# AbbVie-ComputationalGenomics/SAIGEgds

Hardware: AMD Instinct MI355X
Metric: variants/sec seqAssocGLMM_SPA at N=430K; achieved HBM GB/s vs roofline (higher is better)
Workload: dtype f64

## Files before the change

### saigegds_amd/csrc/host_lanes.h

```cpp
extern "C" int sgx_set_option(sgx_handle *h, const char *name, long long value)
{
	if (!h || !name) return fail(SGX_EINVAL, "sgx_set_option: NULL argument");
	const std::string n(name);
	if (n == "score_v1") h->force_v1 = value != 0;
	else if (n == "force_dense") h->force_dense = value != 0;
	else if (n == "spa_exact") h->force_exact = value != 0;
	else if (n == "pipe_mb") { if (value < 0 || value > 65536) return fail(SGX_EINVAL, "pipe_mb out of range"); h->pipe_bytes = (size_t)value << 20; return SGX_OK; }
	else if (n == "spa_abl") h->spa_abl = (int)value;
	else if (n == "guard_exp") { if (value < 0 || value > 300) return fail(SGX_EINVAL, "guard_exp must be 0..300"); h->guard_tol = std::pow(10.0, -(double)value); }
	else if (n == "three_plane") { if (value < -1 || value > 1) return fail(SGX_EINVAL, "three_plane must be -1 (automatic), 0 or 1"); h->dense_opt = (int)value; return SGX_OK; }
	else if (n == "lanes") {
		if (value < 1 || value > 4) return fail(SGX_EINVAL, "lanes must be 1..4");
		if (h->owner) return fail(SGX_EINVAL, "lanes: not on a twin");
		int rc = sgx_sync(h);
		if (rc) return rc;
		for (int i = (int)value - 1; i < 3; i++) if (h->twins[i]) { sgx_free(h->twins[i]); h->twins[i] = nullptr; }
		for (int i = 0; i < (int)value - 1; i++) {
			if (h->twins[i]) continue;
			sgx_handle *t = new sgx_handle();
			t->device = h->device; t->md = h->md; t->mf_ok = h->mf_ok; t->mfe = h->mfe;
			for (int g = 0; g < MF_MAXG; g++) { t->mf[g] = h->mf[g]; t->mf_nbfv[g] = h->mf_nbfv[g]; }
			t->dF = h->dF; t->dX = h->dX; t->dy = h->dy; t->dmu = h->dmu; t->dmu2 = h->dmu2; t->dXM = h->dXM; t->dFl = h->dFl; t->dQ = h->dQ;
			t->shares_model = true; t->owner = h;
			t->force_dense = h->force_dense; t->force_v1 = h->force_v1; t->force_exact = h->force_exact;
			t->spa_abl = h->spa_abl; t->guard_tol = h->guard_tol;
			rc = set_dev(t);
			if (!rc) rc = alloc_workspace(t);
			if (rc) { sgx_free(t); return rc; }
			h->twins[i] = t;
		}
		h->n_lanes = (int)value; h->next_lane = 0; h->last_issued = nullptr;
		return SGX_OK;
	}
	else return fail(SGX_EINVAL, "sgx_set_option: unknown option '%s'", name);
	for (sgx_handle *t : h->twins) if (t) { int rc = sgx_set_option(t, name, value); if (rc) return rc; }
	return SGX_OK;
}

static int sync_lane(sgx_handle *h)
{
	int rc = set_dev(h);
	if (rc) return rc;
	HIPCHK(hipStreamSynchronize(h->stream));
	if (h->pend_dense.active) {
		h->pend_dense.active = false;
		if (h->stats_pending && h->h_counters[2] > 0) {
			rc = launch_pending_dense(h);
			if (rc) return rc;
			HIPCHK(hipStreamSynchronize(h->stream));
		}
	}
	if (h->stats_pending) {
		h->stats.n_spa = (uint64_t)(h->h_counters[0] + h->h_counters[7] - h->h_counters[6] + h->h_counters[5]);
		h->stats.n_valid = (uint64_t)h->h_counters[1];
		h->stats.n_spa_dense = (uint64_t)h->h_counters[2];
		h->stats.n_spa_slow = (uint64_t)h->h_counters[4];
		h->stats.three_plane = h->used_miss ? 1u : 0u;
		h->stats.n_guarded = (uint32_t)h->h_counters[21];
		h->stats.n_unlisted = (uint32_t)h->h_counters[23] - h->stats.n_guarded;
		if (h->chain_ran) {
			sgx_handle *p = h->owner ? h->owner : h;
			const double frac = 64.0 * (double)h->h_counters[22] / ((double)std::max<uint64_t>(1, h->stats.n_variants) * (double)h->md.N);
			const bool over = (uint64_t)h->stats.n_unlisted * 32 > h->stats.n_variants;
			if (!h->used_miss && (frac > SGX_DENSE_ON || over)) p->dense_mode = true;
			else if (h->used_miss && frac < SGX_DENSE_OFF) p->dense_mode = false;
		}
#ifdef SPA5_PROF
		fprintf(stderr, "routing: tier A %d, tier B %d (of them handed on by A: %d), per-variant kernels %d (series list %d, exact list %d), dense %d\n",
			h->h_counters[0], h->h_counters[7], h->h_counters[6], h->h_counters[5], h->h_counters[3], h->h_counters[4], h->h_counters[2]);
		fprintf(stderr, "spa5 phases (10 ns ticks summed over variants): series kernel %d variants: stage %d count %d index %d gather %d series %d (sweep %d sum %d solve %d) | exact kernel %d variants: stage %d count %d index %d gather %d - sweeps %d\n",
			h->h_counters[3], h->h_counters[8], h->h_counters[9], h->h_counters[10], h->h_counters[11], h->h_counters[12], h->h_counters[13], h->h_counters[14], h->h_counters[15],
			h->h_counters[4], h->h_counters[16], h->h_counters[17], h->h_counters[18], h->h_counters[19], h->h_counters[21]);
#endif
		float a = 0, b = 0, c = 0;
		(void)hipEventElapsedTime(&a, h->ev[0], h->ev[1]);
		(void)hipEventElapsedTime(&b, h->ev[1], h->ev[2]);
		(void)hipEventElapsedTime(&c, h->ev[0], h->ev[2]);
		h->stats.ms_score = a; h->stats.ms_spa = b; h->stats.ms_total = c;
		float k = 0;
		if (h->evk_set) (void)hipEventElapsedTime(&k, h->evk[0], h->evk[1]);
		h->stats.ms_kernel = k; h->evk_set = false;
		float l = 0;
		if (h->lists_timed) { (void)hipEventElapsedTime(&l, h->ev_lists, h->ev[0]); h->stats.ms_total += l; }
		h->stats.ms_lists = l; h->lists_timed = false;
		h->stats_pending = false;
		sgx_handle *p = h->owner ? h->owner : h;
		const sgx_stats &x = h->stats;
		p->total.n_variants += x.n_variants; p->total.n_valid += x.n_valid; p->total.n_spa += x.n_spa;
		p->total.n_spa_dense += x.n_spa_dense; p->total.n_spa_slow += x.n_spa_slow;
		p->total.ms_score += x.ms_score; p->total.ms_spa += x.ms_spa; p->total.ms_total += x.ms_total; p->total.ms_kernel += x.ms_kernel;
		p->total.ms_lists += x.ms_lists;
		p->total.score_launches += x.score_launches; p->total.spa_launches += x.spa_launches;
		p->total.three_plane += x.three_plane; p->total.n_unlisted += x.n_unlisted; p->total.n_guarded += x.n_guarded;
		p->total_calls++;
	}
	return SGX_OK;
}

extern "C" int sgx_sync(sgx_handle *h)
{
	if (!h) return fail(SGX_EINVAL, "sgx_sync: NULL handle");
	int rc = sync_lane(h);
	for (sgx_handle *t : h->twins) if (!rc && t) rc = sync_lane(t);
	return rc;
}

extern "C" int sgx_get_stats(sgx_handle *h, sgx_stats *st)
{
	if (!h || !st) return fail(SGX_EINVAL, "sgx_get_stats: NULL argument");
	int rc = sgx_sync(h);
	if (rc) return rc;
	*st = (h->last_issued && h->last_issued != h) ? h->last_issued->stats : h->stats;
	return SGX_OK;
}

extern "C" int sgx_get_stats_total(sgx_handle *h, sgx_stats *st, uint64_t *n_calls, int reset)
{
	if (!h || !st) return fail(SGX_EINVAL, "sgx_get_stats_total: NULL argument");
	int rc = sgx_sync(h);
	if (rc) return rc;
	*st = h->total;
	if (n_calls) *n_calls = h->total_calls;
	if (reset) { h->total = sgx_stats{}; h->total_calls = 0; }
	return SGX_OK;
}
```

### saigegds_amd/csrc/host_spa.h

```cpp


#define FOR_EACH_K(X) X(1) X(2) X(3) X(4) X(5) X(6) X(7) X(8) X(9) X(10) X(11) X(12) X(13) X(14) X(15) X(16)

static dim3 mf_grid(int n_cu, size_t rows, int ntile, int *tps, int vpb = MF_VPB, int wg_per_cu = 2)
{
	const int vt = (int)((rows + vpb - 1) / vpb);
	int sk = std::max(1, (n_cu * wg_per_cu * 4 + vt / 2) / vt);
	sk = std::min(sk, std::max(1, ntile / 24));
	if (sk >= 6) sk = (sk + 7) & ~7;
	sk = std::min(sk, std::max(1, ntile / 2));
	*tps = (ntile + sk - 1) / sk;
	*tps += *tps & 1;
	sk = (ntile + *tps - 1) / *tps;
	return dim3((unsigned)vt, (unsigned)sk);
}

template <int INPUT>
static int launch_spa(sgx_handle *h, RowsRef rr, size_t M, double *out8, bool lazy_dense = false)
{
	const DevModel &md = h->md;
	constexpr int PB = 512;
	hipStream_t st = h->stream;
	h->stats.spa_launches = 0;
	if (!md.quant) {
		const dim3 sgrid((unsigned)std::min<size_t>(M, (size_t)h->spa_grid));
		switch (md.K) {
#define MOMENTS(KK, NCX, TIER, RD)                                                               \
	do {                                                                                         \
		if (INPUT == IN_2BIT)                                                                    \
			hipLaunchKernelGGL((spa4_moments<KK, NCX>), dim3((unsigned)h->n_cu), \
				dim3(WAVE * spa4_waves(KK)), fl, st, rr, md, h->nseg,  \
				TIER, btop, (RD) * h->vcap4, h->vcap4, h->recs, h->counters, h->seg4, h->spa_abl, h->cur5 + 2); \
		else                                                                                     \
			hipLaunchKernelGGL((spa4_moments_ds<KK, NCX, (INPUT == IN_2BIT ? IN_U8 : INPUT)>),   \
				dim3((unsigned)h->n_cu), dim3(WAVE * spa4_waves(KK)), fl, st, (const void *)rr.base, rr.bpv, md, \
				h->nseg, TIER, btop, (RD) * h->vcap4, h->vcap4, h->recs, h->counters, h->seg4, h->cur5 + 2);  \
		hipLaunchKernelGGL((spa4_solve<KK, NCX>), gsolve, dim3(256), 0, st, md, h->nseg, TIER,   \
			btop, (RD) * h->vcap4, h->vcap4, h->recs, h->counters, h->seg4, h->fallback,         \
			h->fb_x2, out8, h->force_dense ? 1 : 0, h->force_exact ? 1 : 0);                     \
	} while (0)
#define CASE(KK)                                                                             \
	case KK:                                                                                 \
		if (h->force_v1 && INPUT != IN_2BIT) {                                               \
			hipLaunchKernelGGL((spa_kernel<KK, PB, INPUT>), sgrid, dim3(PB), 0, st, rr,    \
				md, h->recs, h->counters, 0, (const int *)nullptr, h->scratch,    \
				h->scratch_stride, out8);                                                    \
		} else {                                                                             \
			              \
			const size_t fl = spa4_lds_bytes(KK);                                            \
			if (!h->mom_attr_set[INPUT]) {                                                   \
				const void *fa = INPUT == IN_2BIT ? (const void *)spa4_moments<KK, SPA4_NCA> \
					: (const void *)spa4_moments_ds<KK, SPA4_NCA, (INPUT == IN_2BIT ? IN_U8 : INPUT)>; \
				const void *fb = INPUT == IN_2BIT ? (const void *)spa4_moments<KK, SPA4_NCB> \
					: (const void *)spa4_moments_ds<KK, SPA4_NCB, (INPUT == IN_2BIT ? IN_U8 : INPUT)>; \
				HIPCHK(hipFuncSetAttribute(fa, hipFuncAttributeMaxDynamicSharedMemorySize, (int)fl)); \
				HIPCHK(hipFuncSetAttribute(fb, hipFuncAttributeMaxDynamicSharedMemorySize, (int)fl)); \
				h->mom_attr_set[INPUT] = true;                                               \
			}                                                                                \
			const int nround = (int)((M + h->vcap4 - 1) / h->vcap4);                         \
			const int btop = (int)(2 * M);                                                   \
			const dim3 gsolve((unsigned)std::min((h->vcap4 + 3) / 4, 4 * h->n_cu));    \
			                                    \
			 \
			const size_t rowb5 = (size_t)((md.N + 63) / 64) * 16;                            \
			const size_t l5 = (INPUT == IN_2BIT && rowb5 <= 120 * 1024) ? rowb5 : 0;         \
			const bool small5 = INPUT == IN_2BIT && rowb5 <= 32 * 1024;                      \
			if (l5 > 48 * 1024 && !h->spa5_attr_set[INPUT]) {                                \
				HIPCHK(hipFuncSetAttribute((const void *)spa5_kernel<KK, INPUT, 0, 512>,     \
					hipFuncAttributeMaxDynamicSharedMemorySize, (int)l5));                   \
				HIPCHK(hipFuncSetAttribute((const void *)spa5_kernel<KK, INPUT, 1, 512>,     \
					hipFuncAttributeMaxDynamicSharedMemorySize, (int)l5));                   \
				h->spa5_attr_set[INPUT] = true;                                              \
			}                                                                                \
			const int fx5 = (h->force_exact ? 1 : 0) | (h->spa_abl & ~1);                    \
			for (int rd = 0; rd < nround; rd++) MOMENTS(KK, SPA4_NCA, 0, rd);                \
			for (int rd = 0; rd < nround; rd++) MOMENTS(KK, SPA4_NCB, 1, rd);                \
			 \
			const int only5 = (INPUT == IN_2BIT && rr.cptr != nullptr && (h->spa_abl & 512)) ? 2 : 0; \
			const size_t ws5 = spa5_wg_bytes(md.N);                                          \
			if (small5) {                                                                    \
				 \
				constexpr int IN5 = INPUT == IN_2BIT ? INPUT : IN_2BIT;                      \
				hipLaunchKernelGGL((spa5_kernel<KK, IN5, 0, 128>), dim3((unsigned)h->nwg5), dim3(128), \
					l5, st, rr, md, h->recs, h->counters, h->fb_spa2, h->fb_x2, h->cur5, \
					h->fallback, h->scr5, out8, h->force_dense ? 1 : 0, fx5, l5, only5, ws5, 3); \
				hipLaunchKernelGGL((spa5_kernel<KK, IN5, 1, 128>), dim3((unsigned)h->nwg5), dim3(128), \
					l5, st, rr, md, h->recs, h->counters, h->fb_x2, h->fb_x2, h->cur5 + 1, \
					h->fallback, h->scr5, out8, h->force_dense ? 1 : 0, fx5, l5, only5, ws5, 4); \
			} else {                                                                         \
				hipLaunchKernelGGL((spa5_kernel<KK, INPUT, 0, 512>), dim3((unsigned)h->n_cu), dim3(512), \
					l5, st, rr, md, h->recs, h->counters, h->fb_spa2, h->fb_x2, h->cur5, \
					h->fallback, h->scr5, out8, h->force_dense ? 1 : 0, fx5, l5, only5, ws5, 3); \
				hipLaunchKernelGGL((spa5_kernel<KK, INPUT, 1, 512>), dim3((unsigned)h->n_cu), dim3(512), \
					l5, st, rr, md, h->recs, h->counters, h->fb_x2, h->fb_x2, h->cur5 + 1, \
					h->fallback, h->scr5, out8, h->force_dense ? 1 : 0, fx5, l5, only5, ws5, 4); \
			}                                                                                \
			if (!lazy_dense)                                                                 \
				hipLaunchKernelGGL((spa_kernel<KK, PB, INPUT>), sgrid, dim3(PB), 0, st, rr,  \
					md, h->recs, h->counters, 2, h->fallback, h->scratch,                    \
					h->scratch_stride, out8);                                                \
		}                                                                                    \
		break;
			FOR_EACH_K(CASE)
#undef CASE
#undef MOMENTS
		}
		HIPCHK(hipGetLastError());
		h->stats.spa_launches = (h->force_v1 && INPUT != IN_2BIT) ? 1u : (uint32_t)(4 * ((M + h->vcap4 - 1) / h->vcap4) + 3);
		if (lazy_dense && !(h->force_v1 && INPUT != IN_2BIT)) { h->pend_dense.active = true; h->pend_dense.rr = rr; h->pend_dense.M = M; h->pend_dense.out8 = out8; }
	}
	return SGX_OK;
}

static int launch_pending_dense(sgx_handle *h)
{
	const DevModel &md = h->md;
	const RowsRef rr = h->pend_dense.rr;
	double *out8 = h->pend_dense.out8;
	const dim3 sgrid((unsigned)std::min<size_t>(h->pend_dense.M, (size_t)h->spa_grid));
	switch (md.K) {
#define DCASE(KK) case KK: hipLaunchKernelGGL((spa_kernel<KK, 512, IN_2BIT>), sgrid, dim3(512), 0, h->stream, rr, md, h->recs, \
		h->counters, 2, h->fallback, h->scratch, h->scratch_stride, out8); break;
		FOR_EACH_K(DCASE)
#undef DCASE
	}
	HIPCHK(hipGetLastError());
	return SGX_OK;
}

template <int INPUT>
static int launch_scan(sgx_handle *h, const void *rows, size_t row_bytes, size_t M,
	double *out8, uint8_t *valid)
{
	const DevModel &md = h->md;
	constexpr int SB = 256;
	hipStream_t st = h->stream;
	const RowsRef rr{reinterpret_cast<const uint8_t *>(rows), row_bytes, 0, nullptr, nullptr, nullptr};
	HIPCHK(hipMemsetAsync(h->counters, 0, 24 * sizeof(int), st));
	if (h->cur5) HIPCHK(hipMemsetAsync(h->cur5, 0, 8 * sizeof(int), st));
	HIPCHK(hipEventRecord(h->ev[0], st));
	{
	const dim3 grid((unsigned)M);
		switch (md.K) {
	#define CASE(KK)                                                                             \
		case KK:                                                                                 \
			if (INPUT == IN_2BIT)                                                                \
				hipLaunchKernelGGL((score2b_kernel<2 * KK + 2, SB>), grid, dim3(SB), 0, st,     \
					rr, (int)M, md, h->recs, h->counters, out8, valid, (const int *)nullptr, 0, 0, (int *)nullptr, (int *)nullptr); \
			else if (KK <= 8 && !h->force_v1) {                                                  \
				         \
				constexpr int PT = (KK <= 8) ? 2 * KK + 2 : 4;                                   \
				const int vb = (int)((M + DS_TILE_VB - 1) / DS_TILE_VB);                         \
				int ns = std::max(1, std::min((4 * h->n_cu + vb - 1) / vb, (md.N + 4095) / 4096)); \
				int per = (((md.N + ns - 1) / ns) + 63) & ~63;                                   \
				ns = (md.N + per - 1) / per;                                                     \
				const size_t need = (size_t)ns * M * (3 * PT + 2) * sizeof(double);              \
				if (need > h->ds_part_cap) {                                                     \
					HIPCHK(hipStreamSynchronize(st));                                            \
					if (h->ds_part) HIPCHK(hipFree(h->ds_part));                                 \
					h->ds_part = nullptr; h->ds_part_cap = 0;                                    \
					HIPCHK(hipMalloc((void **)&h->ds_part, need));                               \
					h->ds_part_cap = need;                                                       \
				}                                                                                \
				const dim3 gt((unsigned)vb, (unsigned)ns);                                       \
				if (INPUT == IN_U8)                                                              \
					hipLaunchKernelGGL((score_ds_tile_kernel<PT, uint8_t>), gt, dim3(256), 0, st, \
						(const uint8_t *)rows, (int)M, md, per, h->ds_part);                     \
				else                                                                             \
					hipLaunchKernelGGL((score_ds_tile_kernel<PT, double>), gt, dim3(256), 0, st, \
						(const double *)rows, (int)M, md, per, h->ds_part);                      \
				hipLaunchKernelGGL((score_ds_tile_epilogue<PT>), dim3((unsigned)((M + 255) / 256)), dim3(256), 0, st, \
					(int)M, md, ns, h->ds_part, h->recs, h->counters, out8, valid);              \
			} else if (INPUT == IN_U8)                                                           \
				hipLaunchKernelGGL((score_ds_kernel<2 * KK + 2, SB, uint8_t>), grid, dim3(SB), 0, st, \
					(const uint8_t *)rows, (int)M, md, h->recs, h->counters, out8, valid);      \
			else                                                                                 \
				hipLaunchKernelGGL((score_ds_kernel<2 * KK + 2, SB, double>), grid, dim3(SB), 0, st, \
					(const double *)rows, (int)M, md, h->recs, h->counters, out8, valid);       \
			break;
			FOR_EACH_K(CASE)
	#undef CASE
		default: return fail(SGX_EINVAL, "unsupported K=%d", md.K);
		}
	}
	HIPCHK(hipGetLastError());
	HIPCHK(hipEventRecord(h->ev[1], st));
	h->stats.score_launches = 1;
	h->used_miss = false; h->chain_ran = false;
	int rc = launch_spa<INPUT>(h, rr, M, out8);
	if (rc) return rc;
	HIPCHK(hipEventRecord(h->ev[2], st));
	HIPCHK(hipMemcpyAsync(h->h_counters, h->counters, 24 * sizeof(int), hipMemcpyDeviceToHost, st));
	h->stats.n_variants = M;
	h->stats_pending = true;
	return SGX_OK;
}
```

### saigegds_amd/csrc/kern_spa4.h

```cpp
#pragma once
#include "kern_spa4_tab.h"


#ifndef SPA4_WAVES_LOWK
#define SPA4_WAVES_LOWK 8
#endif
__host__ __device__ constexpr int spa4_waves(int K) { return K <= 8 ? SPA4_WAVES_LOWK : 8; }
#define SPA4_NCA 12
#define SPA4_NCB SPA4_NC
#define SPA4_NSMAX (SPA4_NC + 5)
#define SPA4_TAIL_TOL 1e-10

__device__ __forceinline__ double spa4_fma_svv(double a_sgpr, double x, double c_vgpr)
{
	double r;
	asm("v_fma_f64 %0, %1, %2, %3" : "=v"(r) : "s"(a_sgpr), "v"(x), "v"(c_vgpr));
	return r;
}

__device__ __forceinline__ void spa4_max_abs(double &g, double a)
{
	asm("v_max_f64 %0, %0, |%1|" : "+v"(g) : "v"(a));
}

// ... 341 lines not shown
#pragma unroll
			for (int a = 0; a < NS - 1; a++) acc[a] = 0;
			auto dosage = [&](int j) -> double {
				const int i = s_lo + j * WAVE + lane;
				if (i >= N) return 0.0;
				if (INPUT == IN_U8) {
					const uint8_t v = row[i];
					return (v == 0xFF) ? imp : (minus ? 2.0 - (double)v : (double)v);
				} else {
					const double v = reinterpret_cast<const double *>(row)[i];
					return !isfinite(v) ? imp : (minus ? 2.0 - v : v);
				}
			};
			double gn = dosage(0);
			for (int j = 0; j < nstep; j++) {
				const double G = gn;
				if (j + 1 < nstep) gn = dosage(j + 1);
				if (G != 0) {
					const double *x = tab + (size_t)(j * WAVE + lane) * KP;
					double bb = 0;
#pragma unroll
					for (int a = 0; a < K; a++) bb = fma(x[a], c[a], bb);
					const double mui = x[K];
					const double adj = (G - bb) * inv;
					const double u = mui * (1 - mui);
					acc[0] = fma(mui, G, acc[0]);
					acc[1] += bb;
					acc[2] += fmax(adj, 0.0); acc[3] += fmin(adj, 0.0);
					acc[4] = fma(adj, mui, acc[4]);
					acc[5] = fma(adj * adj, u, acc[5]);
					spa4_max_abs(gmax, adj);
					spa4_cum_terms<NC>(adj * ts, u, 1 - 2 * mui, &acc[6]);
				}
			}
			const int idx = wave_reduce_scatter(acc, lane);
			gmax = wave_max_nonneg_to_last(gmax);
			const size_t base = ((size_t)(vb + vl) * nseg + seg) * NS;
			if (!(lane & (NS - 1 > 16 ? 1 : 3)) && idx < NS - 1) segpart[base + idx] = acc[0];
			if (lane == WAVE - 1) segpart[base + (NS - 1)] = gmax;
		}
	}
	spa4_queue_done(cursor);
}

template <int NC>
struct Spa4Series {
	double k1, k2;
	double kp[NC - 2];
	double ts, gmax;
};

template <int NC>
__device__ __forceinline__ bool spa4_eval(const Spa4Series<NC> &S, double xmax, double t, double &K1s, double &K2s, double &K0s)
{
	const double its = 1 / S.ts, tau = t * its;
	double p0 = 0, p1 = 0, p2 = 0;
#pragma unroll
	for (int n = NC; n >= 3; n--) {
		const double kn = S.kp[n - 3];
		p0 = fma(p0, tau, kn);
		p1 = fma(p1, tau, (double)n * kn);
		p2 = fma(p2, tau, (double)(n * (n - 1)) * kn);
	}
	const double tau2 = tau * tau;
	K0s = fma(t, S.k1, fma(0.5 * t * t, S.k2, p0 * tau2 * tau));
	K1s = S.k1 + fma(t, S.k2, p1 * tau2 * its);
	K2s = fma(p2 * tau, its * its, S.k2);
	double tp = tau;
#pragma unroll
	for (int k = 1; k < NC - 3; k++) tp *= tau;
	const double tail = (fabs((double)(NC * (NC - 1)) * S.kp[NC - 3] * tp * tau) +
		fabs((double)((NC - 1) * (NC - 2)) * S.kp[NC - 4] * tp)) * its * its;
	return S.gmax * fabs(t) <= xmax && tail <= SPA4_TAIL_TOL * fabs(K2s) && isfinite(K2s);
}

template <int NC>
__device__ __forceinline__ bool spa4_root(const Spa4Series<NC> &S, double xmax, double q, double NAmu, double NAsigma, RootState &s)
{
	root_begin(s, q, 0, 0);
	root_feed(s, S.k1, S.k2, NAmu, NAsigma, 0.0, true);
	while (s.active) {
		double K1s, K2s, K0s;
		if (!spa4_eval(S, xmax, s.tnew, K1s, K2s, K0s)) return false;
		root_feed(s, K1s, K2s, NAmu, NAsigma, K0s, true);
	}
	return true;
}

template <int K, int NC>
__device__ __forceinline__ void spa4_solve_one(const DevModel &md, int nseg, int tier, int btop, int v0, int vcap, int v, int lane,
	SpaRec *__restrict__ recs, int *__restrict__ counters, const double *__restrict__ segpart,
	int *__restrict__ fb_dense, int *__restrict__ fb_exact, double *__restrict__ out8, int force_dense, int force_exact);

template <int K, int NC>
__global__ void __launch_bounds__(256)
spa4_solve(DevModel md, int nseg, int tier, int btop, int v0, int vcap, SpaRec *__restrict__ recs, int *__restrict__ counters,
	const double *__restrict__ segpart, int *__restrict__ fb_dense, int *__restrict__ fb_exact,
	double *__restrict__ out8, int force_dense, int force_exact)
{
	const int lane = threadIdx.x & (WAVE - 1);
	const int nflag = min(counters[tier ? 7 : 0] - v0, vcap);
	for (int v = (blockIdx.x * blockDim.x + threadIdx.x) / WAVE; v < nflag; v += gridDim.x * blockDim.x / WAVE)
		spa4_solve_one<K, NC>(md, nseg, tier, btop, v0, vcap, v, lane, recs, counters, segpart, fb_dense, fb_exact, out8,
			force_dense, force_exact);
}

template <int K, int NC>
__device__ __forceinline__ void spa4_solve_one(const DevModel &md, int nseg, int tier, int btop, int v0, int vcap, int v, int lane,
	SpaRec *__restrict__ recs, int *__restrict__ counters, const double *__restrict__ segpart,
	int *__restrict__ fb_dense, int *__restrict__ fb_exact, double *__restrict__ out8, int force_dense, int force_exact)
{
	constexpr int NS = NC + 5;
	const int ri = spa4_rec(tier, btop, v0 + v);
	const SpaRec r = recs[ri];
	double a[NS];
#pragma unroll
	for (int x = 0; x < NS; x++) a[x] = 0;
	for (int s = lane; s < nseg; s += WAVE) {
		const double *p = segpart + ((size_t)v * nseg + s) * NS;
#pragma unroll
		for (int x = 0; x < NS - 1; x++) a[x] += p[x];
		a[NS - 1] = fmax(a[NS - 1], p[NS - 1]);
	}
#pragma unroll
	for (int x = 0; x < NS - 1; x++) a[x] = wave_sum(a[x]);
#pragma unroll
	for (int o = 32; o > 0; o >>= 1) a[NS - 1] = fmax(a[NS - 1], __shfl_xor(a[NS - 1], o, WAVE));
	if (lane > 1) return;
	const double inv = 1 / sqrt(r.AC2);
	double xmu_c = 0, xsum_c = 0;
#pragma unroll
	for (int x = 0; x < K; x++) { xmu_c = fma(md.Xmu[x], r.c[x], xmu_c); xsum_c = fma(md.Xsum[x], r.c[x], xsum_c); }
	const double Tstat = r.S * inv;
	const double var2 = r.var2 / r.AC2, var1 = var2 * md.r;
	const double m1 = (a[0] - xmu_c) * inv;
	const double qtilde = Tstat / sqrt(var1) * sqrt(var2) + m1;
	const double sdev = qtilde - m1, qinv = -sdev + m1;
	const double pn_in = d_pchisq1_upper(sdev * sdev / var2);
	if (fabs(qtilde - m1) / sqrt(var2) < 2.0) {
		if (lane == 0) spa_write_row(r, Tstat, var1, pn_in, true, out8);
		return;
	}
	const double nb = (xsum_c - a[1]) * inv;
	const double L = a[2] + fmax(-nb, 0.0), U = a[3] + fmin(-nb, 0.0);
	const double mar = 1e-9 * (fabs(L) + fabs(U) + fabs(qtilde) + fabs(qinv));
	if (force_dense || !(qtilde < L - mar && qtilde > U + mar && qinv < L - mar && qinv > U + mar)) {
		if (lane == 0) fb_dense[atomicAdd(&counters[2], 1)] = ri;
		return;
	}
	Spa4Series<NC> S;
	S.k1 = a[4]; S.k2 = a[5]; S.ts = r.tscale; S.gmax = a[NS - 1];
#pragma unroll
	for (int x = 0; x < NC - 2; x++) S.kp[x] = a[6 + x];
	const double NAmu = m1 - a[4], NAsigma = var2 - a[5];
	const double qmine = lane == 0 ? qtilde : qinv;
	RootState sm;
	const bool ok_mine = !force_exact && spa4_root(S, md.spa_xmax, qmine, NAmu, NAsigma, sm);
	double p_mine = 0;
	if (ok_mine && sm.converged) p_mine = lugannani_rice(sm.root, sm.Kcur, sm.K2cur, qmine, NAmu, NAsigma);
	const int st_mine = (ok_mine ? 1 : 0) | (ok_mine && sm.converged ? 2 : 0);
	const double p_other = __shfl(p_mine, 1, WAVE);
	const int st_other = __shfl(st_mine, 1, WAVE);
	if (lane != 0) return;
	if (!(st_mine & 1) || !(st_other & 1)) {
		if (tier == 0 && !force_exact) {
			const int slot = atomicAdd(&counters[7], 1);
			atomicAdd(&counters[6], 1);
			recs[btop - 1 - slot] = r;
		} else {
			fb_exact[atomicAdd(&counters[4], 1)] = ri;
		}
		return;
	}
	double pval;
	bool converged = true;
	if ((st_mine & 2) && (st_other & 2)) {
		pval = fabs(p_mine) + fabs(p_other);
		if (pval != 0 && pn_in / pval > 1000) pval = pn_in;
	} else {
		pval = pn_in;
		converged = false;
	}
	spa_write_row(r, Tstat, var1, pval, converged, out8);
}


#define SPA5_BIG 2048

__device__ __forceinline__ void cgf_terms_rt(double g, double m, double t, bool with_k, double &k1, double &k2, double &k0)
{
	const double om = 1 - m, mg = m * g, c2 = om * mg * g;
	const double e = fast_exp(-g * t);
	const double d = fma(om, e, m);
	const double rr = isfinite(d) ? fast_rcp(d) : 0.0;
	k1 = fma(mg, rr, k1);
	const double tt = c2 * e * rr * rr;
	if (isfinite(tt)) k2 += tt;
	if (with_k) k0 += cgf_korg_term(g, m, t, d, om);
}

__host__ __device__ inline size_t spa5_wg_bytes(int N) { return (((size_t)N + 63) & ~(size_t)63) * (16 + 4); }

template <int BLOCK>
__device__ __noinline__ void spa5_cum_sweep(const double2 *__restrict__ glist, int nnz, double ts, double *kp_out)
{
	constexpr int NC = SPA4_NCB;
	double kp[NC - 1];
#pragma unroll
	for (int a = 0; a < NC - 1; a++) kp[a] = 0;
	double2 gn = (int)threadIdx.x < nnz ? glist[threadIdx.x] : make_double2(0.0, 0.5);
	for (int k = threadIdx.x; k < nnz; k += BLOCK) {
		const double2 gm = gn;
		if (k + BLOCK < nnz) gn = glist[k + BLOCK];
		const double mui = gm.y;
		spa4_cum_terms<NC>(gm.x * ts, mui * (1 - mui), 1 - 2 * mui, kp);
		kp[NC - 2] = fmax(kp[NC - 2], fabs(gm.x));
	}
#pragma unroll
	for (int a = 0; a < NC - 1; a++) kp_out[a] = kp[a];
}

__device__ __noinline__ int spa5_series_solve(const double *arg, const SpaRec *__restrict__ rec, double *__restrict__ out8)
{
	constexpr int NC = SPA4_NCB;
	Spa4Series<NC> S;
#pragma unroll
	for (int a = 0; a < NC - 2; a++) S.kp[a] = arg[a];
	S.k1 = arg[NC - 2]; S.k2 = arg[NC - 1]; S.ts = arg[NC]; S.gmax = arg[NC + 1];
	const double xmax = arg[NC + 2], qtilde = arg[NC + 3], qinv = arg[NC + 4], NAmu = arg[NC + 5], NAsigma = arg[NC + 6];
	const double pn_in = arg[NC + 7], Tstat = arg[NC + 8], var1 = arg[NC + 9];
	RootState s1, s2;
	if (!spa4_root(S, xmax, qtilde, NAmu, NAsigma, s1) || !spa4_root(S, xmax, qinv, NAmu, NAsigma, s2)) return 0;
	double pval;
	bool converged = true;
	if (s1.converged && s2.converged) {
		const double p1 = lugannani_rice(s1.root, s1.Kcur, s1.K2cur, qtilde, NAmu, NAsigma);
		const double p2 = lugannani_rice(s2.root, s2.Kcur, s2.K2cur, qinv, NAmu, NAsigma);
		pval = fabs(p1) + fabs(p2);
		if (pval != 0 && pn_in / pval > 1000) pval = pn_in;
	} else {
		pval = pn_in;
		converged = false;
	}
	const SpaRec rr = *rec;
	spa_write_row(rr, Tstat, var1, pval, converged, out8);
	return 1;
}

template <int BLOCK>
__device__ __forceinline__ bool spa5_series(const double2 *__restrict__ glist, int nnz, double ts, double xmax,
	double k1, double k2, double qtilde, double qinv, double NAmu, double NAsigma, double pn_in,
	double Tstat, double var1, const SpaRec *__restrict__ rec, double *__restrict__ out8, double *sh, int *sh_flag, int *prof = nullptr)
{
	constexpr int NC = SPA4_NCB;
	double kp[NC - 1];
#ifdef SPA5_PROF
	long long tp_ = wall_clock64();
#define SPA5_TS(ph) do { if (threadIdx.x == 0) { const long long now_ = wall_clock64(); atomicAdd(&prof[ph], (int)(now_ - tp_)); tp_ = now_; } } while (0)
#else
#define SPA5_TS(ph) do { } while (0)
#endif
	spa5_cum_sweep<BLOCK>(glist, nnz, ts, kp);
	SPA5_TS(0);
	constexpr int NWV = BLOCK / WAVE;
	double gmax = kp[NC - 2];
	const int lane = threadIdx.x & (WAVE - 1), wv = threadIdx.x / WAVE;
	double kr[NC - 2];
#pragma unroll
	for (int a = 0; a < NC - 2; a++) kr[a] = kp[a];
	const int idx = wave_reduce_scatter(kr, lane);
#pragma unroll
	for (int o = 32; o > 0; o >>= 1) gmax = fmax(gmax, __shfl_xor(gmax, o, WAVE));
	double *part = sh + NC + 16;
	if (!(lane & 3) && idx < NC - 2) part[idx * NWV + wv] = kr[0];
	if (lane == 1) part[(NC - 2) * NWV + wv] = gmax;
	__syncthreads();
	double *arg = sh;
	if (threadIdx.x < NC - 2) {
		double t = 0;
		for (int w = 0; w < NWV; w++) t += part[threadIdx.x * NWV + w];
		arg[threadIdx.x] = t;
	}
	__syncthreads();
	SPA5_TS(1);
	if (threadIdx.x == 0) {
		for (int w = 0; w < NWV; w++) gmax = fmax(gmax, part[(NC - 2) * NWV + w]);
		arg[NC - 2] = k1; arg[NC - 1] = k2; arg[NC] = ts; arg[NC + 1] = gmax; arg[NC + 2] = xmax;
		arg[NC + 3] = qtilde; arg[NC + 4] = qinv; arg[NC + 5] = NAmu; arg[NC + 6] = NAsigma;
		arg[NC + 7] = pn_in; arg[NC + 8] = Tstat; arg[NC + 9] = var1;
		*sh_flag = spa5_series_solve(arg, rec, out8);
	}
	SPA5_TS(2);
	__syncthreads();
	const bool done = *sh_flag != 0;
	__syncthreads();
	return done;
}

#ifndef SPA5_REG_WAVES
#define SPA5_REG_WAVES 2
#endif
#define SPA5_WAVES_PER_SIMD(BLOCK) ((BLOCK) == 512 ? SPA5_REG_WAVES : ((BLOCK) / 64 + 3) / 4)
#ifdef SPA5_PROF
#define SPA5_T(ph) do { if (tid == 0) { const long long now_ = wall_clock64(); atomicAdd(&counters[8 + 8 * MODE + (ph)], (int)(now_ - tprev_)); tprev_ = now_; } } while (0)
#else
#define SPA5_T(ph) do { } while (0)
#endif
template <int K, int INPUT, int MODE, int BLOCK>
__global__ void __launch_bounds__(BLOCK, SPA5_WAVES_PER_SIMD(BLOCK))
spa5_kernel(RowsRef rr, DevModel md, const SpaRec *__restrict__ recs,
	int *__restrict__ counters, const int *__restrict__ todo, int *__restrict__ todo_next, int *__restrict__ cursor,
	int *__restrict__ fb_dense, uint8_t *__restrict__ scratch, double *__restrict__ out8, int force_dense, int force_exact,
	size_t lds_row_bytes, int only, size_t wg_stride, int nslot)
{
	constexpr int KP = (K + 2) & ~1, NW = BLOCK / WAVE;
	extern __shared__ __attribute__((aligned(16))) uint8_t fill_smem[];
	uint4 *rows_lds = reinterpret_cast<uint4 *>(fill_smem);
	__shared__ double sh[SPA4_NCB * NW + SPA4_NCB + 16];
	__shared__ int sh_flag;
	__shared__ int shi[NW];
	__shared__ int sh_vi, sh_v;
	__shared__ SpaRec sh_rec;
	const int N = md.N, tid = threadIdx.x, lane = tid & (WAVE - 1), wid = tid / WAVE;
	double2 *glist = reinterpret_cast<double2 *>(scratch + (size_t)blockIdx.x * wg_stride);
	uint32_t *ilist = reinterpret_cast<uint32_t *>(glist + (((size_t)N + 63) & ~(size_t)63));
	const int ntodo = counters[nslot];
	const int nvec = INPUT == IN_2BIT ? (int)(min((size_t)((N + 63) >> 6) * 16, rr_row_bytes(rr)) / 16) : (N + 63) >> 6;
	const int per = ((nvec + NW - 1) / NW + WAVE - 1) & ~(WAVE - 1);
	for (;;) {
		__syncthreads();
		if (tid < WAVE) {
			int vi0 = 0;
			if (tid == 0) vi0 = atomicAdd(cursor, 1);
			vi0 = __builtin_amdgcn_readfirstlane(vi0);
			int v0 = -1;
			if (vi0 < 2 * ntodo) {
				v0 = todo[vi0 < ntodo ? vi0 : vi0 - ntodo];
				const double *src = reinterpret_cast<const double *>(recs + v0);
				for (int i = tid; i < (int)(sizeof(SpaRec) / 8); i += WAVE) reinterpret_cast<double *>(&sh_rec)[i] = src[i];
			}
			if (tid == 0) { sh_vi = vi0; sh_v = v0; }
		}
		__syncthreads();
		const int vi = sh_vi;
		if (vi >= 2 * ntodo) break;
#ifdef SPA5_PROF
		long long tprev_ = wall_clock64();
#endif
		const bool big_round = vi < ntodo;
		const int v = sh_v;
		const SpaRec &r = sh_rec;
		if ((r.nnz > SPA5_BIG) != big_round) continue;
		auto row_piece = [&](int p) -> uint4 { return *reinterpret_cast<const uint4 *>(rr.base + rr_piece(rr, (size_t)r.j, (size_t)p)); };
		const uint32_t zx = r.minus ? 0xAAAAAAAAu : 0u;
		const double lut0 = r.lut[0], lut1 = r.lut[1], lut2 = r.lut[2], lut3 = r.lut[3];
		const bool listed = INPUT == IN_2BIT && only != 2 && rr.cptr != nullptr && rr.corient[r.j] == (r.minus ? 2 : 1);
		const uint32_t *il = listed ? rr.cidx + rr.cptr[r.j] : ilist;
		int nnz = listed ? r.nnz : 0;
		if (!listed) {
			const bool staged = INPUT == IN_2BIT && lds_row_bytes >= (size_t)nvec * 16;
			if (staged) {
				constexpr int UN = 8;
				for (int p0 = tid; p0 < nvec; p0 += UN * BLOCK) {
					uint4 t[UN];
	#pragma unroll
					for (int j = 0; j < UN; j++) { const int p = p0 + j * BLOCK; t[j] = p < nvec ? row_piece(p) : make_uint4(0u, 0u, 0u, 0u); }
	#pragma unroll
					for (int j = 0; j < UN; j++) { const int p = p0 + j * BLOCK; if (p < nvec) rows_lds[p] = t[j]; }
				}
				__syncthreads();
			}
			SPA5_T(0);
			auto masks = [&](int p, uint32_t (&ww)[4], uint32_t (&z)[4]) -> int {
				int cnt = 0;
				if (INPUT == IN_2BIT) {
					uint4 w = make_uint4(0u, 0u, 0u, 0u);
					if (p < nvec) w = staged ? rows_lds[p] : row_piece(p);
					ww[0] = w.x; ww[1] = w.y; ww[2] = w.z; ww[3] = w.w;
	#pragma unroll
					for (int k = 0; k < 4; k++) { z[k] = nz_fields((ww[k] ^ zx) & keep_mask(N - p * 64 - 16 * k)); cnt += __popc(z[k]); }
				} else {
					z[0] = z[1] = z[2] = z[3] = 0;
					if (p < nvec) {
						for (int s2 = 0; s2 < 64; s2++) {
							const int i = p * 64 + s2;
							if (i < N && load_dosage<INPUT>(rr, i, r) != 0) { z[s2 >> 5] |= 1u << (s2 & 31); cnt++; }
						}
					}
				}
				return cnt;
			};
			int cnt_w = 0;
			for (int it = 0; it < per; it += WAVE) {
				uint32_t ww[4], z[4];
				cnt_w += masks(wid * per + it + lane, ww, z);
			}
			cnt_w = wave_sum_i(cnt_w);
			if (lane == 0) shi[wid] = cnt_w;
			__syncthreads();
			int o_w = 0;
	#pragma unroll
			for (int w = 0; w < NW; w++) { if (w < wid) o_w += shi[w]; nnz += shi[w]; }
			SPA5_T(1);
			for (int it = 0; it < per; it += WAVE) {
				uint32_t ww[4], z[4];
				const int p = wid * per + it + lane;
				const int cnt = masks(p, ww, z);
				if (!__ballot(cnt != 0)) continue;
				int incl = cnt;
	#pragma unroll
				for (int o = 1; o < WAVE; o <<= 1) {
					const int up = __shfl_up(incl, o, WAVE);
					if (lane >= o) incl += up;
				}
				int o2 = o_w + incl - cnt;
				o_w += __shfl(incl, WAVE - 1, WAVE);
				if (INPUT == IN_2BIT) {
	#pragma unroll
					for (int k = 0; k < 4; k++) {
						uint32_t zz = z[k];
						while (zz) {
							const int b = __ffs(zz) - 1;
							zz &= zz - 1;
							ilist[o2++] = (uint32_t)(p * 64 + 16 * k + (b >> 1)) | (((ww[k] >> b) & 3u) << 30);
						}
					}
				} else {
	#pragma unroll
					for (int k = 0; k < 2; k++) {
						uint32_t zz = z[k];
						while (zz) {
							const int b = __ffs(zz) - 1;
							zz &= zz - 1;
							ilist[o2++] = (uint32_t)(p * 64 + 32 * k + b);
						}
					}
				}
			}
			__syncthreads();
			SPA5_T(2);
		}
		const double inv = 1 / sqrt(r.AC2);
		double c[K];
#pragma unroll
		for (int a = 0; a < K; a++) c[a] = r.c[a];
		double a6[6] = {0, 0, 0, 0, 0, 0};
		constexpr int UNG = K <= 4 ? 4 : 2;
		for (int k0 = tid; k0 < ((force_exact & 128) ? 0 : nnz); k0 += UNG * BLOCK) {
			uint32_t e[UNG];
			double xv[UNG][KP];
#pragma unroll
			for (int j = 0; j < UNG; j++) e[j] = (k0 + j * BLOCK < nnz) ? il[k0 + j * BLOCK] : 0u;
#pragma unroll
			for (int j = 0; j < UNG; j++) {
				const double *x = md.XM + (size_t)(e[j] & 0x3FFFFFFFu) * KP;
#pragma unroll
				for (int a = 0; a < KP; a += 2) {
					const double2 t2 = *reinterpret_cast<const double2 *>(x + a);
					xv[j][a] = t2.x; xv[j][a + 1] = t2.y;
				}
			}
#pragma unroll
			for (int j = 0; j < UNG; j++) {
				const int k = k0 + j * BLOCK;
				if (k >= nnz) continue;
				const uint32_t code = e[j] >> 30;
				const double G = INPUT == IN_2BIT ? ((code & 2u) ? ((code & 1u) ? lut3 : lut2) : ((code & 1u) ? lut1 : lut0))
					: load_dosage<INPUT>(rr, (int)(e[j] & 0x3FFFFFFFu), r);
				double b = 0;
#pragma unroll
				for (int a = 0; a < K; a++) b = fma(xv[j][a], c[a], b);
				const double mui = xv[j][K];
				const double adj = (G - b) * inv;
				glist[k] = make_double2(adj, mui);
				a6[0] = fma(mui, G, a6[0]);
				a6[1] += b;
				if (adj > 0) a6[2] += adj; else a6[3] += adj;
				a6[4] = fma(adj, mui, a6[4]);
				a6[5] = fma(adj * adj, mui * (1 - mui), a6[5]);
			}
		}
		block_sum<6, BLOCK>(a6, sh);
		SPA5_T(3);
		double xmu_c = 0, xsum_c = 0;
#pragma unroll
		for (int a = 0; a < K; a++) { xmu_c = fma(md.Xmu[a], c[a], xmu_c); xsum_c = fma(md.Xsum[a], c[a], xsum_c); }
		const double m1 = (a6[0] - xmu_c) * inv;
		const double Tstat = r.S * inv;
		const double var2 = r.var2 / r.AC2, var1 = var2 * md.r;
		const double qtilde = Tstat / sqrt(var1) * sqrt(var2) + m1;
		const double sdev = qtilde - m1, qinv = -sdev + m1;
		const double pn_in = d_pchisq1_upper(sdev * sdev / var2);
		double pval;
		bool converged = true;
		if (fabs(qtilde - m1) / sqrt(var2) < 2.0) {
			pval = pn_in;
		} else {
			const double nb = (xsum_c - a6[1]) * inv;
			const double L = a6[2] + fmax(-nb, 0.0), U = a6[3] + fmin(-nb, 0.0);
			const double mar = 1e-9 * (fabs(L) + fabs(U) + fabs(qtilde) + fabs(qinv));
			if (force_dense || !(qtilde < L - mar && qtilde > U + mar && qinv < L - mar && qinv > U + mar)) {
				if (tid == 0) fb_dense[atomicAdd(&counters[2], 1)] = v;
				continue;
			}
			const double NAmu = m1 - a6[4], NAsigma = var2 - a6[5];
			if (MODE == 0) {
				if ((force_exact & 1) || !spa5_series<BLOCK>(glist, nnz, r.tscale, md.spa_xmax, a6[4], a6[5], qtilde, qinv, NAmu, NAsigma,
						pn_in, Tstat, var1, &sh_rec, out8, sh, &sh_flag, counters + 13)) {
					if (tid == 0) todo_next[atomicAdd(&counters[4], 1)] = v;
				}
				SPA5_T(4);
				continue;
			}
			RootState s1, s2;
			root_begin(s1, qtilde, L, U);
			root_begin(s2, qinv, L, U);
			root_feed(s1, a6[4], a6[5], NAmu, NAsigma, 0.0, true);
			root_feed(s2, a6[4], a6[5], NAmu, NAsigma, 0.0, true);
			auto sweep = [&](bool a1, bool a2, bool k1w, bool k2w, double t1, double t2, double (&sv)[6]) {
#pragma unroll
				for (int a = 0; a < 6; a++) sv[a] = 0;
				double2 gn = tid < nnz ? glist[tid] : make_double2(0.0, 0.5);
				for (int k0 = tid; k0 < nnz; k0 += BLOCK) {
					const double2 gm = gn;
					if (k0 + BLOCK < nnz) gn = glist[k0 + BLOCK];
					if (a1) cgf_terms_rt(gm.x, gm.y, t1, k1w, sv[0], sv[1], sv[2]);
					if (a2) cgf_terms_rt(gm.x, gm.y, t2, k2w, sv[3], sv[4], sv[5]);
				}
				block_sum<6, BLOCK>(sv, sh);
			};
			while ((s1.active || s2.active) && !(force_exact & 64)) {
				const bool a1 = s1.active, a2 = s2.active, k1w = s1.want_k, k2w = s2.want_k;
				double sv[6];
				sweep(a1, a2, k1w, k2w, s1.tnew, s2.tnew, sv);
				if (a1) root_feed(s1, sv[0], sv[1], NAmu, NAsigma, sv[2], k1w);
				if (a2) root_feed(s2, sv[3], sv[4], NAmu, NAsigma, sv[5], k2w);
			}
			if (s1.converged && s2.converged) {
				if (!(s1.k_ok && s2.k_ok)) {
					double sv[6];
					sweep(!s1.k_ok, !s2.k_ok, true, true, s1.root, s2.root, sv);
					if (!s1.k_ok) s1.Kcur = sv[2];
					if (!s2.k_ok) s2.Kcur = sv[5];
				}
				const double p1 = lugannani_rice(s1.root, s1.Kcur, s1.K2cur, qtilde, NAmu, NAsigma);
				const double p2 = lugannani_rice(s2.root, s2.Kcur, s2.K2cur, qinv, NAmu, NAsigma);
				pval = fabs(p1) + fabs(p2);
				if (pval != 0 && pn_in / pval > 1000) pval = pn_in;
			} else {
				pval = pn_in;
				converged = false;
			}
		}
		if (tid == 0) spa_write_row(r, Tstat, var1, pval, converged, out8);
		SPA5_T(5);
	}
}
```

Measured before the change: 17.64 million.

## Merge series and exact SPA passes into one kernel launch with in-place fallthrough

The two launches of spa5_kernel (series mode, then exact mode over a todo list) become one kernel that reads both the exact and series lists. When the series expansion fails, the variant goes straight to the exact root-finding sweeps in the same workgroup, reusing the already gathered glist and moments instead of re-staging the variant in a second launch. This removes one launch and the repeated gather/count work for the variants that fall through. In exchange, the series and exact paths now share one workgroup's work distribution and can load-imbalance, and a last-block atomic updates counters[4] so the host statistics stay consistent.

Result: no change. 17.70 million, median of 6 (+0.3%).

```diff
diff --git a/saigegds_amd/csrc/host_lanes.h b/saigegds_amd/csrc/host_lanes.h
--- a/saigegds_amd/csrc/host_lanes.h
+++ b/saigegds_amd/csrc/host_lanes.h
@@ -68,9 +68,9 @@
 #ifdef SPA5_PROF
 		fprintf(stderr, "routing: tier A %d, tier B %d (of them handed on by A: %d), per-variant kernels %d (series list %d, exact list %d), dense %d\n",
 			h->h_counters[0], h->h_counters[7], h->h_counters[6], h->h_counters[5], h->h_counters[3], h->h_counters[4], h->h_counters[2]);
-		fprintf(stderr, "spa5 phases (10 ns ticks summed over variants): series kernel %d variants: stage %d count %d index %d gather %d series %d (sweep %d sum %d solve %d) | exact kernel %d variants: stage %d count %d index %d gather %d - sweeps %d\n",
-			h->h_counters[3], h->h_counters[8], h->h_counters[9], h->h_counters[10], h->h_counters[11], h->h_counters[12], h->h_counters[13], h->h_counters[14], h->h_counters[15],
-			h->h_counters[4], h->h_counters[16], h->h_counters[17], h->h_counters[18], h->h_counters[19], h->h_counters[21]);
+		fprintf(stderr, "spa5 phases (10 ns ticks summed over variants): %d variants (series list %d, of them on to the exact sweeps %d): stage %d count %d index %d gather %d series %d (sweep %d sum %d solve %d) exact sweeps %d (%d variants)\n",
+			h->h_counters[3] + h->h_counters[4] - h->h_counters[20], h->h_counters[3], h->h_counters[20], h->h_counters[8], h->h_counters[9], h->h_counters[10],
+			h->h_counters[11], h->h_counters[12], h->h_counters[13], h->h_counters[14], h->h_counters[15], h->h_counters[16], h->h_counters[4]);
 #endif
 		float a = 0, b = 0, c = 0;
 		(void)hipEventElapsedTime(&a, h->ev[0], h->ev[1]);
diff --git a/saigegds_amd/csrc/host_spa.h b/saigegds_amd/csrc/host_spa.h
--- a/saigegds_amd/csrc/host_spa.h
+++ b/saigegds_amd/csrc/host_spa.h
@@ -66,9 +66,7 @@
 			const size_t l5 = (INPUT == IN_2BIT && rowb5 <= 120 * 1024) ? rowb5 : 0;         \
 			const bool small5 = INPUT == IN_2BIT && rowb5 <= 32 * 1024;                      \
 			if (l5 > 48 * 1024 && !h->spa5_attr_set[INPUT]) {                                \
-				HIPCHK(hipFuncSetAttribute((const void *)spa5_kernel<KK, INPUT, 0, 512>,     \
-					hipFuncAttributeMaxDynamicSharedMemorySize, (int)l5));                   \
-				HIPCHK(hipFuncSetAttribute((const void *)spa5_kernel<KK, INPUT, 1, 512>,     \
+				HIPCHK(hipFuncSetAttribute((const void *)spa5_kernel<KK, INPUT, 512>,        \
 					hipFuncAttributeMaxDynamicSharedMemorySize, (int)l5));                   \
 				h->spa5_attr_set[INPUT] = true;                                              \
 			}                                                                                \
@@ -78,22 +76,17 @@
 			 \
 			const int only5 = (INPUT == IN_2BIT && rr.cptr != nullptr && (h->spa_abl & 512)) ? 2 : 0; \
 			const size_t ws5 = spa5_wg_bytes(md.N);                                          \
+			 \
 			if (small5) {                                                                    \
 				 \
 				constexpr int IN5 = INPUT == IN_2BIT ? INPUT : IN_2BIT;                      \
-				hipLaunchKernelGGL((spa5_kernel<KK, IN5, 0, 128>), dim3((unsigned)h->nwg5), dim3(128), \
-					l5, st, rr, md, h->recs, h->counters, h->fb_spa2, h->fb_x2, h->cur5, \
-					h->fallback, h->scr5, out8, h->force_dense ? 1 : 0, fx5, l5, only5, ws5, 3); \
-				hipLaunchKernelGGL((spa5_kernel<KK, IN5, 1, 128>), dim3((unsigned)h->nwg5), dim3(128), \
-					l5, st, rr, md, h->recs, h->counters, h->fb_x2, h->fb_x2, h->cur5 + 1, \
-					h->fallback, h->scr5, out8, h->force_dense ? 1 : 0, fx5, l5, only5, ws5, 4); \
+				hipLaunchKernelGGL((spa5_kernel<KK, IN5, 128>), dim3((unsigned)h->nwg5), dim3(128), \
+					l5, st, rr, md, h->recs, h->counters, h->fb_spa2, h->fb_x2, h->cur5, h->cur5 + 1, \
+					h->fallback, h->scr5, out8, h->force_dense ? 1 : 0, fx5, l5, only5, ws5); \
 			} else {                                                                         \
-				hipLaunchKernelGGL((spa5_kernel<KK, INPUT, 0, 512>), dim3((unsigned)h->n_cu), dim3(512), \
-					l5, st, rr, md, h->recs, h->counters, h->fb_spa2, h->fb_x2, h->cur5, \
-					h->fallback, h->scr5, out8, h->force_dense ? 1 : 0, fx5, l5, only5, ws5, 3); \
-				hipLaunchKernelGGL((spa5_kernel<KK, INPUT, 1, 512>), dim3((unsigned)h->n_cu), dim3(512), \
-					l5, st, rr, md, h->recs, h->counters, h->fb_x2, h->fb_x2, h->cur5 + 1, \
-					h->fallback, h->scr5, out8, h->force_dense ? 1 : 0, fx5, l5, only5, ws5, 4); \
+				hipLaunchKernelGGL((spa5_kernel<KK, INPUT, 512>), dim3((unsigned)h->n_cu), dim3(512), \
+					l5, st, rr, md, h->recs, h->counters, h->fb_spa2, h->fb_x2, h->cur5, h->cur5 + 1, \
+					h->fallback, h->scr5, out8, h->force_dense ? 1 : 0, fx5, l5, only5, ws5); \
 			}                                                                                \
 			if (!lazy_dense)                                                                 \
 				hipLaunchKernelGGL((spa_kernel<KK, PB, INPUT>), sgrid, dim3(PB), 0, st, rr,  \
@@ -106,7 +99,7 @@
 #undef MOMENTS
 		}
 		HIPCHK(hipGetLastError());
-		h->stats.spa_launches = (h->force_v1 && INPUT != IN_2BIT) ? 1u : (uint32_t)(4 * ((M + h->vcap4 - 1) / h->vcap4) + 3);
+		h->stats.spa_launches = (h->force_v1 && INPUT != IN_2BIT) ? 1u : (uint32_t)(4 * ((M + h->vcap4 - 1) / h->vcap4) + 2);
 		if (lazy_dense && !(h->force_v1 && INPUT != IN_2BIT)) { h->pend_dense.active = true; h->pend_dense.rr = rr; h->pend_dense.M = M; h->pend_dense.out8 = out8; }
 	}
 	return SGX_OK;
diff --git a/saigegds_amd/csrc/kern_spa4.h b/saigegds_amd/csrc/kern_spa4.h
--- a/saigegds_amd/csrc/kern_spa4.h
+++ b/saigegds_amd/csrc/kern_spa4.h
@@ -667,16 +667,37 @@
 #endif
 #define SPA5_WAVES_PER_SIMD(BLOCK) ((BLOCK) == 512 ? SPA5_REG_WAVES : ((BLOCK) / 64 + 3) / 4)
 #ifdef SPA5_PROF
-#define SPA5_T(ph) do { if (tid == 0) { const long long now_ = wall_clock64(); atomicAdd(&counters[8 + 8 * MODE + (ph)], (int)(now_ - tprev_)); tprev_ = now_; } } while (0)
+#define SPA5_T(ph) do { if (tid == 0) { const long long now_ = wall_clock64(); atomicAdd(&counters[(ph) == 5 ? 16 : 8 + (ph)], (int)(now_ - tprev_)); tprev_ = now_; } } while (0)
 #else
 #define SPA5_T(ph) do { } while (0)
 #endif
-template <int K, int INPUT, int MODE, int BLOCK>
+struct Spa5Scalars { double m1, Tstat, var2, var1, qtilde, qinv, pn_in, L, U; };
+template <int K>
+__device__ __forceinline__ Spa5Scalars spa5_scalars(const DevModel &md, const SpaRec &r, const double (&a6)[6])
+{
+	Spa5Scalars z;
+	const double inv = 1 / sqrt(r.AC2);
+	double xmu_c = 0, xsum_c = 0;
+#pragma unroll
+	for (int a = 0; a < K; a++) { xmu_c = fma(md.Xmu[a], r.c[a], xmu_c); xsum_c = fma(md.Xsum[a], r.c[a], xsum_c); }
+	z.m1 = (a6[0] - xmu_c) * inv;
+	z.Tstat = r.S * inv;
+	z.var2 = r.var2 / r.AC2; z.var1 = z.var2 * md.r;
+	z.qtilde = z.Tstat / sqrt(z.var1) * sqrt(z.var2) + z.m1;
+	const double sdev = z.qtilde - z.m1;
+	z.qinv = -sdev + z.m1;
+	z.pn_in = d_pchisq1_upper(sdev * sdev / z.var2);
+	const double nb = (xsum_c - a6[1]) * inv;
+	z.L = a6[2] + fmax(-nb, 0.0); z.U = a6[3] + fmin(-nb, 0.0);
+	return z;
+}
+
+template <int K, int INPUT, int BLOCK>
 __global__ void __launch_bounds__(BLOCK, SPA5_WAVES_PER_SIMD(BLOCK))
 spa5_kernel(RowsRef rr, DevModel md, const SpaRec *__restrict__ recs,
-	int *__restrict__ counters, const int *__restrict__ todo, int *__restrict__ todo_next, int *__restrict__ cursor,
-	int *__restrict__ fb_dense, uint8_t *__restrict__ scratch, double *__restrict__ out8, int force_dense, int force_exact,
-	size_t lds_row_bytes, int only, size_t wg_stride, int nslot)
+	int *__restrict__ counters, const int *__restrict__ series, const int *__restrict__ exact, int *__restrict__ cursor,
+	int *__restrict__ done, int *__restrict__ fb_dense, uint8_t *__restrict__ scratch, double *__restrict__ out8, int force_dense,
+	int force_exact, size_t lds_row_bytes, int only, size_t wg_stride)
 {
 	constexpr int KP = (K + 2) & ~1, NW = BLOCK / WAVE;
 	extern __shared__ __attribute__((aligned(16))) uint8_t fill_smem[];
@@ -686,10 +707,11 @@
 	__shared__ int shi[NW];
 	__shared__ int sh_vi, sh_v;
 	__shared__ SpaRec sh_rec;
+	__shared__ double sh_a6[6];
 	const int N = md.N, tid = threadIdx.x, lane = tid & (WAVE - 1), wid = tid / WAVE;
 	double2 *glist = reinterpret_cast<double2 *>(scratch + (size_t)blockIdx.x * wg_stride);
 	uint32_t *ilist = reinterpret_cast<uint32_t *>(glist + (((size_t)N + 63) & ~(size_t)63));
-	const int ntodo = counters[nslot];
+	const int nexact = counters[4], ntodo = nexact + counters[3];
 	const int nvec = INPUT == IN_2BIT ? (int)(min((size_t)((N + 63) >> 6) * 16, rr_row_bytes(rr)) / 16) : (N + 63) >> 6;
 	const int per = ((nvec + NW - 1) / NW + WAVE - 1) & ~(WAVE - 1);
 	for (;;) {
@@ -700,7 +722,8 @@
 			vi0 = __builtin_amdgcn_readfirstlane(vi0);
 			int v0 = -1;
 			if (vi0 < 2 * ntodo) {
-				v0 = todo[vi0 < ntodo ? vi0 : vi0 - ntodo];
+				const int q = vi0 < ntodo ? vi0 : vi0 - ntodo;
+				v0 = q < nexact ? exact[q] : series[q - nexact];
 				const double *src = reinterpret_cast<const double *>(recs + v0);
 				for (int i = tid; i < (int)(sizeof(SpaRec) / 8); i += WAVE) reinterpret_cast<double *>(&sh_rec)[i] = src[i];
 			}
@@ -713,6 +736,7 @@
 		long long tprev_ = wall_clock64();
 #endif
 		const bool big_round = vi < ntodo;
+		const bool on_series = (big_round ? vi : vi - ntodo) >= nexact;
 		const int v = sh_v;
 		const SpaRec &r = sh_rec;
 		if ((r.nnz > SPA5_BIG) != big_round) continue;
@@ -847,39 +871,36 @@
 		}
 		block_sum<6, BLOCK>(a6, sh);
 		SPA5_T(3);
-		double xmu_c = 0, xsum_c = 0;
-#pragma unroll
-		for (int a = 0; a < K; a++) { xmu_c = fma(md.Xmu[a], c[a], xmu_c); xsum_c = fma(md.Xsum[a], c[a], xsum_c); }
-		const double m1 = (a6[0] - xmu_c) * inv;
-		const double Tstat = r.S * inv;
-		const double var2 = r.var2 / r.AC2, var1 = var2 * md.r;
-		const double qtilde = Tstat / sqrt(var1) * sqrt(var2) + m1;
-		const double sdev = qtilde - m1, qinv = -sdev + m1;
-		const double pn_in = d_pchisq1_upper(sdev * sdev / var2);
+		Spa5Scalars z = spa5_scalars<K>(md, r, a6);
 		double pval;
 		bool converged = true;
-		if (fabs(qtilde - m1) / sqrt(var2) < 2.0) {
-			pval = pn_in;
+		if (fabs(z.qtilde - z.m1) / sqrt(z.var2) < 2.0) {
+			pval = z.pn_in;
 		} else {
-			const double nb = (xsum_c - a6[1]) * inv;
-			const double L = a6[2] + fmax(-nb, 0.0), U = a6[3] + fmin(-nb, 0.0);
-			const double mar = 1e-9 * (fabs(L) + fabs(U) + fabs(qtilde) + fabs(qinv));
-			if (force_dense || !(qtilde < L - mar && qtilde > U + mar && qinv < L - mar && qinv > U + mar)) {
+			const double mar = 1e-9 * (fabs(z.L) + fabs(z.U) + fabs(z.qtilde) + fabs(z.qinv));
+			if (force_dense || !(z.qtilde < z.L - mar && z.qtilde > z.U + mar && z.qinv < z.L - mar && z.qinv > z.U + mar)) {
 				if (tid == 0) fb_dense[atomicAdd(&counters[2], 1)] = v;
 				continue;
 			}
-			const double NAmu = m1 - a6[4], NAsigma = var2 - a6[5];
-			if (MODE == 0) {
-				if ((force_exact & 1) || !spa5_series<BLOCK>(glist, nnz, r.tscale, md.spa_xmax, a6[4], a6[5], qtilde, qinv, NAmu, NAsigma,
-						pn_in, Tstat, var1, &sh_rec, out8, sh, &sh_flag, counters + 13)) {
-					if (tid == 0) todo_next[atomicAdd(&counters[4], 1)] = v;
-				}
+			if (on_series) {
+				if (tid == 0) {
+#pragma unroll
+					for (int a = 0; a < 6; a++) sh_a6[a] = a6[a];
+				}
+				const bool sdone = !(force_exact & 1) && spa5_series<BLOCK>(glist, nnz, r.tscale, md.spa_xmax, a6[4], a6[5], z.qtilde,
+					z.qinv, z.m1 - a6[4], z.var2 - a6[5], z.pn_in, z.Tstat, z.var1, &sh_rec, out8, sh, &sh_flag, counters + 13);
 				SPA5_T(4);
-				continue;
-			}
+				if (sdone) continue;
+				if (tid == 0) atomicAdd(&counters[20], 1);
+				if (force_exact & 1) __syncthreads();
+#pragma unroll
+				for (int a = 0; a < 6; a++) a6[a] = sh_a6[a];
+				z = spa5_scalars<K>(md, sh_rec, a6);
+			}
+			const double qtilde = z.qtilde, qinv = z.qinv, NAmu = z.m1 - a6[4], NAsigma = z.var2 - a6[5];
 			RootState s1, s2;
-			root_begin(s1, qtilde, L, U);
-			root_begin(s2, qinv, L, U);
+			root_begin(s1, qtilde, z.L, z.U);
+			root_begin(s2, qinv, z.L, z.U);
 			root_feed(s1, a6[4], a6[5], NAmu, NAsigma, 0.0, true);
 			root_feed(s2, a6[4], a6[5], NAmu, NAsigma, 0.0, true);
 			auto sweep = [&](bool a1, bool a2, bool k1w, bool k2w, double t1, double t2, double (&sv)[6]) {
@@ -911,13 +932,20 @@
 				const double p1 = lugannani_rice(s1.root, s1.Kcur, s1.K2cur, qtilde, NAmu, NAsigma);
 				const double p2 = lugannani_rice(s2.root, s2.Kcur, s2.K2cur, qinv, NAmu, NAsigma);
 				pval = fabs(p1) + fabs(p2);
-				if (pval != 0 && pn_in / pval > 1000) pval = pn_in;
+				if (pval != 0 && z.pn_in / pval > 1000) pval = z.pn_in;
 			} else {
-				pval = pn_in;
+				pval = z.pn_in;
 				converged = false;
 			}
 		}
-		if (tid == 0) spa_write_row(r, Tstat, var1, pval, converged, out8);
+		if (tid == 0) spa_write_row(r, z.Tstat, z.var1, pval, converged, out8);
 		SPA5_T(5);
 	}
-}
+	if (tid == 0) {
+		__threadfence();
+		if (atomicAdd(done, 1) == (int)gridDim.x - 1) {
+			__threadfence();
+			atomicAdd(&counters[4], atomicAdd(&counters[20], 0));
+		}
+	}
+}
```
